# renegade-fi/mpc-jellyfish

Measured on AMD Instinct MI355X. Metric: msm_g1_scalar_pairs_per_s, higher is better.
Workload: dtype u32 (381-bit Fq as 14 x 29-bit limbs, Montgomery)

## Files before the change

mpc-jellyfish_amd/csrc/constants.cuh:

```cuda
#pragma once
#include <cstdint>

namespace mzk {

struct BlsFr {
    static constexpr int N = 8;
    static constexpr int BITS = 255;
    static constexpr uint32_t INV = 0xffffffffu;
    static constexpr uint32_t MOD[8] = {0x00000001u, 0xffffffffu, 0xfffe5bfeu, 0x53bda402u, 0x09a1d805u, 0x3339d808u, 0x299d7d48u, 0x73eda753u};
    static constexpr uint32_t R1[8] = {0xfffffffeu, 0x00000001u, 0x00034802u, 0x5884b7fau, 0xecbc4ff5u, 0x998c4fefu, 0xacc5056fu, 0x1824b159u};
    static constexpr uint32_t R2[8] = {0xf3f29c6du, 0xc999e990u, 0x87925c23u, 0x2b6cedcbu, 0x7254398fu, 0x05d31496u, 0x9f59ff11u, 0x0748d9d9u};
    static constexpr uint32_t ROOT[8] = {0x5f0e466au, 0xb9b58d8cu, 0x1819d7ecu, 0x5b1b4c80u, 0x52a31e64u, 0x0af53ae3u, 0x19e9b27bu, 0x5bf3addau};
    static constexpr uint32_t GENERATOR[8] = {0xfffffff1u, 0x0000000eu, 0x00189c0fu, 0x17e363d3u, 0x6f8457b0u, 0xff9c5787u, 0x8fc5a8c4u, 0x35133220u};
    static constexpr int TWO_ADICITY = 32;
};

struct BnFr {
    static constexpr int N = 8;
    static constexpr int BITS = 254;
    static constexpr uint32_t INV = 0xefffffffu;
    static constexpr uint32_t MOD[8] = {0xf0000001u, 0x43e1f593u, 0x79b97091u, 0x2833e848u, 0x8181585du, 0xb85045b6u, 0xe131a029u, 0x30644e72u};
    static constexpr uint32_t R1[8] = {0x4ffffffbu, 0xac96341cu, 0x9f60cd29u, 0x36fc7695u, 0x7879462eu, 0x666ea36fu, 0x9a07df2fu, 0x0e0a77c1u};
    static constexpr uint32_t R2[8] = {0xae216da7u, 0x1bb8e645u, 0xe35c59e3u, 0x53fe3ab1u, 0x53bb8085u, 0x8c49833du, 0x7f4e44a5u, 0x0216d0b1u};
    static constexpr uint32_t ROOT[8] = {0x80d13d9cu, 0x636e7355u, 0x2445ffd6u, 0xa22bf374u, 0x1eb203d8u, 0x56452ac0u, 0x2963f9e7u, 0x1860ef94u};
// ... 106 lines not shown
    static constexpr uint32_t XR2[9] = {0x059bac10u, 0x0d1503a3u, 0x018016b8u, 0x10ab0ca8u, 0x02632639u, 0x02c0169fu, 0x169bfd53u, 0x11869d4cu, 0x002a11a6u};
    static constexpr uint32_t XPINV[9] = {0x1b799c77u, 0x016fc3e8u, 0x0d654d9eu, 0x030535c2u, 0x0257f612u, 0x1a17f3e6u, 0x0e509d40u, 0x090dceeeu, 0x100a85ddu};
    static constexpr uint32_t XRM[8] = {0x0f6b5c04u, 0x751d5b0fu, 0xe6d91549u, 0x5edd77f4u, 0x422a9d60u, 0x1422c907u, 0xd2402342u, 0x1982b46du};
    static constexpr long long SRC = 346695ll;
    static constexpr int XPAD_MULT = 1;
    static constexpr uint32_t XSUB2[9] = {0x30f9fa8eu, 0x2208c16cu, 0x38e5469du, 0x25aa45a0u, 0x2b0bb2efu, 0x25b68180u, 0x214dc281u, 0x3cb84c67u, 0x0060c89bu};
    static constexpr uint32_t XSUB8[9] = {0x43e7ea38u, 0x482305b4u, 0x43951a76u, 0x56a91685u, 0x4c2ecbbeu, 0x56da0603u, 0x45370a06u, 0x52e1319eu, 0x01832271u};
    static constexpr uint32_t XSUB32[9] = {0x8f9fa8e0u, 0x808c16d4u, 0x8e5469ddu, 0x9aa45a18u, 0x90bb2efeu, 0x9b681811u, 0x94dc281eu, 0x8b84c67cu, 0x060c89cau};
    static constexpr uint32_t XSUB64[9] = {0x5f3f51c0u, 0x41182daeu, 0x5ca8d3c0u, 0x5548b436u, 0x41765e03u, 0x56d03029u, 0x49b85043u, 0x57098cffu, 0x0c19139au};
    static constexpr int XKXY = 8;
    static constexpr uint32_t XSUB_XY[9] = {0x43e7ea38u, 0x482305b4u, 0x43951a76u, 0x56a91685u, 0x4c2ecbbeu, 0x56da0603u, 0x45370a06u, 0x52e1319eu, 0x01832271u};
    static constexpr uint32_t XSUB_PQ[9] = {0x81f3f51cu, 0x841182d7u, 0x91ca8d38u, 0x8b548b3fu, 0x961765dcu, 0x8b6d02feu, 0x829b8500u, 0x997098ccu, 0x00c19135u};
    static constexpr uint32_t XSUB_2S[9] = {0x41f3f51cu, 0x441182d9u, 0x51ca8d3au, 0x4b548b41u, 0x561765deu, 0x4b6d0300u, 0x429b8502u, 0x597098ceu, 0x00c19137u};
};

}
```

mpc-jellyfish_amd/csrc/gen_constants.py:

```python
import os

FIELDS = {}

def limbs32(x, n):
    return [(x >> (32 * i)) & 0xFFFFFFFF for i in range(n)]

def carr(name, vals):
    return "    static constexpr uint32_t %s[%d] = {%s};" % (name, len(vals), ", ".join("0x%08xu" % v for v in vals))

def field_struct(name, p, n32, extra=(), tail=()):
    R = 1 << (32 * n32)
    out = ["struct %s {" % name,
           "    static constexpr int N = %d;            // 32-bit limbs" % n32,
           "    static constexpr int BITS = %d;" % p.bit_length(),
           "    static constexpr uint32_t INV = 0x%08xu;  // -p^-1 mod 2^32" % ((-pow(p, -1, 1 << 32)) % (1 << 32)),
           carr("MOD", limbs32(p, n32)),
           carr("R1", limbs32(R % p, n32)) + "   // Montgomery one",
           carr("R2", limbs32(R * R % p, n32)) + "   // R^2 mod p"]
    for k, v in extra:
        out.append(carr(k, limbs32(v * R % p, n32)))
    out.extend(tail)
    out.append("};")
    return "\n".join(out)

# ... 72 lines not shown
    out.append("    static constexpr int XKXY = %d;           // accumulator invariant: X, Y < XKXY * p" % kxy)
    out.append(arr("XSUB_XY", spread(kxy, p, n29, 1), "%dp: minus an accumulator coordinate (limbs < 2^30 - 1)" % kxy))
    out.append(arr("XSUB_PQ", spread(kpq, p, n29, 2), "%dp: minus PPP + 2Q (limbs < 2^31 - 3)" % kpq))
    out.append(arr("XSUB_2S", spread(k2s, p, n29, 1), "%dp: minus 2S (limbs < 2^30 - 1)" % k2s))
    out.append("};")
    return "\n".join(out)

out.append(fx_struct("BlsFrX", "BlsFr", bls_r, 8, 9))
out.append("")
out.append(fx_struct("BnFrX", "BnFr", bn_r, 8, 9))
out.append("")
out.append(fx_struct("BlsFqX", "BlsFq", bls_q, 12, 14, endo_beta=pow(2, (bls_q - 1) // 3, bls_q)))
out.append("")
out.append(fx_struct("BnFqX", "BnFq", bn_q, 8, 9, ec_pads=(8, 4, 4)))
out.append("")
out.append("}  // namespace mzk")
open(os.path.join(os.path.dirname(os.path.abspath(__file__)), "constants.cuh"), "w").write("\n".join(out) + "\n")
print("wrote constants.cuh")
```

mpc-jellyfish_amd/csrc/msm.cuh:

```cuda
#pragma once
#include <hip/hip_runtime.h>

#include "ec.cuh"
#include "ecx.cuh"

namespace mzk {

constexpr int MSM_THREADS = 256;
constexpr int MSM_ACC_THREADS = 128;
constexpr uint32_t MSM_HEAVY_PER_THREAD = 16;
constexpr uint32_t MSM_HEAVY_RUN = MSM_ACC_THREADS * MSM_HEAVY_PER_THREAD;
constexpr uint32_t MSM_HEAVY_FANIN = MSM_ACC_THREADS * 32;
constexpr int MSM_HEAVY_COUNTERS = 6;
__host__ __device__ inline bool msm_is_heavy(uint32_t count, uint32_t cap) { return count > cap + MSM_HEAVY_RUN; }

inline int msm_choose_window(unsigned long long n) {
    int lg = 0;
    while ((1ull << (lg + 1)) <= n) lg++;
    int c = lg - 2;
    if (c < 4) c = 4;
    if (c > 16) c = 16;
    return c;
}
inline int msm_num_windows(int scalar_bits, int c) { return (scalar_bits + 1 + c - 1) / c; }
// ... 240 lines not shown
};

template <class X>
__device__ __forceinline__ void load_words(uint32_t* dst, const uint32_t* __restrict__ src, int n_words) {
    for (int i = 0; i < n_words / 4; i++) {
        const uint4 v = reinterpret_cast<const uint4*>(src)[i];
        dst[4 * i] = v.x; dst[4 * i + 1] = v.y; dst[4 * i + 2] = v.z; dst[4 * i + 3] = v.w;
    }
}

template <class X>
struct EcFx {
    using Field = X;
    using Aff = AffineX<X>;
    using Pt = XYZZX<X>;
    static constexpr int AFF_WORDS = 2 * X::XN, PT_WORDS = 4 * X::XN;
    static_assert((4 * X::XN) % 4 == 0 && (2 * X::XN) % 2 == 0, "points are whole 16-byte / 8-byte words");
    static __device__ __forceinline__ Aff load_aff(const uint32_t* __restrict__ bases, unsigned long long idx) {
        uint32_t w[AFF_WORDS];
        if constexpr (AFF_WORDS % 4 == 0) {
            const uint4* src = reinterpret_cast<const uint4*>(bases + idx * AFF_WORDS);
#pragma unroll
            for (int i = 0; i < AFF_WORDS / 4; i++) {
                const uint4 v = src[i];
                w[4 * i] = v.x; w[4 * i + 1] = v.y; w[4 * i + 2] = v.z; w[4 * i + 3] = v.w;
            }
        } else {
            const uint2* src = reinterpret_cast<const uint2*>(bases + idx * AFF_WORDS);
#pragma unroll
            for (int i = 0; i < AFF_WORDS / 2; i++) {
// ... 23 lines not shown
    }
    static __device__ __forceinline__ void store_pt(uint32_t* __restrict__ buf, unsigned long long idx, const Pt& p) {
        uint32_t w[PT_WORDS];
#pragma unroll
        for (int i = 0; i < X::XN; i++) {
            w[i] = p.x.l[i]; w[X::XN + i] = p.y.l[i]; w[2 * X::XN + i] = p.zz.l[i]; w[3 * X::XN + i] = p.zzz.l[i];
        }
        uint4* dst = reinterpret_cast<uint4*>(buf + idx * PT_WORDS);
#pragma unroll
        for (int i = 0; i < PT_WORDS / 4; i++) dst[i] = make_uint4(w[4 * i], w[4 * i + 1], w[4 * i + 2], w[4 * i + 3]);
    }
    static __device__ __forceinline__ Pt inf() { return Pt::inf(); }
    static __device__ __forceinline__ Pt madd(const Pt& a, const Aff& q, bool negate) { return xyzzx_madd(a, q, negate); }
    static __device__ __forceinline__ Pt add(const Pt& a, const Pt& b) { return xyzzx_add(a, b); }
    static __device__ __forceinline__ XYZZ<Fp<X>> to_boundary(const Pt& p) { return xyzzx_to_boundary(p); }
};

template <class X>
__global__ __launch_bounds__(MSM_THREADS) void srs_to_internal_kernel(const uint32_t* __restrict__ xy, unsigned long long n, uint32_t* __restrict__ out) {
    const unsigned long long i = (unsigned long long)blockIdx.x * MSM_THREADS + threadIdx.x;
    if (i >= n) return;
    const Fp<X> x = load_fp<X>(xy + i * 2 * X::N), y = load_fp<X>(xy + i * 2 * X::N + X::N);
    const Fx<X> fx = fx_from_boundary<X>(x), fy = fx_from_boundary<X>(y);
    uint32_t* dst = out + i * 2 * X::XN;
#pragma unroll
    for (int k = 0; k < X::XN; k++) { dst[k] = fx.l[k]; dst[X::XN + k] = fy.l[k]; }
}

template <class EC>
__global__ __launch_bounds__(MSM_ACC_THREADS) void msm_accumulate_kernel(const uint32_t* __restrict__ bases, unsigned long long n,
                                                                          const uint32_t* __restrict__ offs, const uint32_t* __restrict__ hist,
// ... 44 lines not shown
    typename EC::Pt acc = EC::inf();
    for (uint32_t k = part; k < cnt; k += S) {
        const uint32_t e = list[k];
        acc = EC::madd(acc, EC::load_aff(bases, e & 0x7fffffffu), (e >> 31) != 0);
    }
    if (whole) {
        const bool empty = acc.is_inf();
        occ[t] = empty ? 0 : 1;
        if (!empty) EC::store_pt(buckets, t, acc);
    } else {
        EC::store_pt(sub, u, acc);
    }
}
template <class EC>
__device__ __forceinline__ void pt_lds_put(uint32_t* lds, int slot, const typename EC::Pt& p) {
    constexpr int N = EC::Field::XN;
#pragma unroll
    for (int i = 0; i < N; i++) {
        lds[i * MSM_ACC_THREADS + slot] = p.x.l[i];
        lds[(N + i) * MSM_ACC_THREADS + slot] = p.y.l[i];
        lds[(2 * N + i) * MSM_ACC_THREADS + slot] = p.zz.l[i];
        lds[(3 * N + i) * MSM_ACC_THREADS + slot] = p.zzz.l[i];
    }
}
template <class EC>
__device__ __forceinline__ typename EC::Pt pt_lds_get(const uint32_t* lds, int slot) {
    constexpr int N = EC::Field::XN;
    typename EC::Pt p;
#pragma unroll
    for (int i = 0; i < N; i++) {
        p.x.l[i] = lds[i * MSM_ACC_THREADS + slot];
        p.y.l[i] = lds[(N + i) * MSM_ACC_THREADS + slot];
        p.zz.l[i] = lds[(2 * N + i) * MSM_ACC_THREADS + slot];
        p.zzz.l[i] = lds[(3 * N + i) * MSM_ACC_THREADS + slot];
    }
    return p;
}
template <class EC, bool ONE_SET>
__global__ __launch_bounds__(MSM_ACC_THREADS) void msm_split_combine_kernel(const uint32_t* __restrict__ sub, unsigned long long n_buckets, int log_split,
                                                                             const uint32_t* __restrict__ order, unsigned long long rank0,
                                                                             uint32_t* __restrict__ buckets, uint8_t* __restrict__ occ) {
    __shared__ uint32_t lds[MSM_ACC_THREADS * EC::PT_WORDS];
// ... 317 lines not shown
        const uint32_t h = M >> lvl;
        const uint32_t items = (uint32_t)lvl * h;
        for (uint32_t r = threadIdx.x; r < items; r += 256) {
            const uint32_t seg = r / h, i = r % h;
            const unsigned long long base = w * M + (seg ? (M >> seg) : 0u);
            fold_one<EC>(buckets, occ, base + i, base + h + i);
        }
        __threadfence_block();
        __syncthreads();
    }
    if (collect && (int)threadIdx.x <= log_m) collect_set<EC>(buckets, occ, M, log_m, w, collect, (int)threadIdx.x);
}

template <class EC>
__device__ __forceinline__ void fold_one_quad(uint32_t* buckets, uint8_t* occ, unsigned long long ia, unsigned long long ib, int role) {
    using X = typename EC::Field;
    constexpr int XN = X::XN;
    if (!occ[ib]) return;
    uint32_t* pa = buckets + ia * EC::PT_WORDS + role * XN;
    const uint32_t* pb = buckets + ib * EC::PT_WORDS + role * XN;
    Fx<X> cb;
#pragma unroll
    for (int i = 0; i < XN; i++) cb.l[i] = pb[i];
    if (!occ[ia]) {
#pragma unroll
        for (int i = 0; i < XN; i++) pa[i] = cb.l[i];
        occ[ia] = 1;
        return;
    }
    Fx<X> ca;
#pragma unroll
    for (int i = 0; i < XN; i++) ca.l[i] = pa[i];
    const Fx<X> r = xyzzx_add_quad<X>(ca, cb, role);
#pragma unroll
    for (int i = 0; i < XN; i++) pa[i] = r.l[i];
}
template <class EC>
__global__ __launch_bounds__(MSM_ACC_THREADS) void msm_fold_quad_kernel(uint32_t* buckets, uint8_t* occ, uint32_t M, uint32_t h, int nseg, int n_win) {
    const unsigned long long t = ((unsigned long long)blockIdx.x * MSM_ACC_THREADS + threadIdx.x) >> 2;
    const int role = threadIdx.x & 3;
    const unsigned long long per_win = (unsigned long long)nseg * h;
    if (t >= per_win * n_win) return;
    const unsigned long long w = t / per_win, r = t % per_win;
    const uint32_t seg = (uint32_t)(r / h), i = (uint32_t)(r % h);
    const unsigned long long base = w * M + (seg ? (M >> seg) : 0u);
    fold_one_quad<EC>(buckets, occ, base + i, base + h + i, role);
}
constexpr int MSM_TAIL_QUAD_THREADS = 512;
// ... 287 lines not shown
```

mpc-jellyfish_amd/csrc/msm.hip:

```cpp
#include <algorithm>
#include <chrono>
#include <thread>
#include <vector>

#include <cmath>
#include <cstdlib>

#include "internal.hpp"
#include "hostfp.hpp"
#include "host_tail.hpp"
#include "msm.cuh"
#include "msm_pre.cuh"

namespace mzk {
std::atomic<bool> g_msm_precompute{true};
namespace {

struct MsmItem {
    const uint32_t* d_bases;
    const uint32_t* d_scalars;
    uint64_t n;
    uint32_t* out_xyz;
    uint64_t base_off;
};
// ... 491 lines not shown
        if (!p0)
            for (auto& it : run) it.d_bases = plain_table + it.base_off * aff_words;
        for (int attempt = 0;; attempt++) {
            const int32_t rc = msm_group_dev<FR, EC>(run.data(), j - i, c, is_mont, p0 ? pre : PreInfo{}, st);
            cur().last_attempts = (uint32_t)attempt + 1;
            if (rc == MSM_RETRY && attempt < 8) continue;
            if (rc == MSM_RETRY) { set_error("MSM heavy-bucket scratch: no fit after 8 attempts"); return MZK_ERR_UNSUPPORTED; }
            MZK_TRY(rc);
            break;
        }
        i = j;
    }
    return MZK_OK;
}

template <class X>
int32_t srs_build_pre_t(Srs& s, hipStream_t st) {
    using EC = EcFx<X>;
    int lg = 0;
    while ((2ull << lg) <= s.n) lg++;
    int c;
    if (s.curve == MZK_CURVE_BLS12_381) c = lg <= 17 ? 16 : 20;
    else c = lg <= 15 ? 15 : (lg <= 19 ? 17 : 20);
    if (const char* force = std::getenv("MZK_PRE_C")) {
        const int f = std::atoi(force);
        if (f >= 8 && f <= 22) c = f;
    }
    const int W = msm_num_windows(256, c);
    const size_t level = (size_t)s.n * EC::AFF_WORDS;
    size_t free_b = 0, total_b = 0;
    HIP_TRY(hipMemGetInfo(&free_b, &total_b));
    size_t budget = free_b / 2;
    if (const char* b = std::getenv("MZK_MSM_TABLE_BUDGET")) budget = std::min<size_t>(budget, (size_t)std::strtoull(b, nullptr, 10));
    if ((size_t)W * level * 4 > budget) { s.pre_c = -1; return MZK_OK; }
    HIP_TRY(hipMalloc((void**)&s.d_pre, (size_t)W * level * 4));
    HIP_TRY(hipStreamSynchronize(st));
    const auto t_build = std::chrono::steady_clock::now();
    HIP_TRY(hipMemcpyAsync(s.d_pre, s.d_int, level * 4, hipMemcpyDeviceToDevice, st));
    const unsigned long long threads = (s.n + 3) / 4;
    for (int w = 1; w < W; w++)
        hipLaunchKernelGGL((pre_next_level_kernel<X>), dim3((unsigned)((threads + 127) / 128)), dim3(128), 0, st,
                           s.d_pre + (size_t)(w - 1) * level, s.d_pre + (size_t)w * level, (unsigned long long)s.n, c);
    HIP_TRY(hipGetLastError());
    HIP_TRY(hipStreamSynchronize(st));
    s.pre_build_ms = std::chrono::duration<double, std::milli>(std::chrono::steady_clock::now() - t_build).count();
    s.pre_c = c;
    s.pre_levels = W;
    return MZK_OK;
}
}
int32_t srs_build_pre(Srs& s, hipStream_t st) {
    if (s.d_pre || s.pre_c < 0 || !s.d_int) return MZK_OK;
    return s.curve == MZK_CURVE_BLS12_381 ? srs_build_pre_t<BlsFqX>(s, st) : srs_build_pre_t<BnFqX>(s, st);
}

int32_t msm_dispatch(const Srs& s, uint64_t base_offset, const uint32_t* d_scalars, uint64_t n, int is_mont, uint32_t* out, hipStream_t st) {
    const uint32_t* sc[1] = {d_scalars};
    return msm_batch_dispatch(s, 1, sc, &n, &base_offset, is_mont, out, st);
}

int32_t msm_batch_dispatch(const Srs& s, uint32_t n_polys, const uint32_t* const* d_scalars, const uint64_t* lens, const uint64_t* base_offsets,
                           int is_mont, uint32_t* out_xyz, hipStream_t st) {
    const int fw = fq_words(s.curve);
    const bool bls = s.curve == MZK_CURVE_BLS12_381;
    const size_t aff_words = bls ? (size_t)EcFx<BlsFqX>::AFF_WORDS : (size_t)EcFx<BnFqX>::AFF_WORDS;
    const uint32_t* table = s.d_int;
    if (!table) { set_error("SRS has no internal table"); return MZK_ERR_BAD_HANDLE; }
    std::vector<MsmItem> items(n_polys);
    bool want_pre = false;
    for (uint32_t i = 0; i < n_polys; i++) {
        const uint64_t off = base_offsets ? base_offsets[i] : 0;
        if (off > s.n || lens[i] > s.n - off) {
            set_error("MSM longer than the registered SRS (poly degree larger than allowed)");
            return MZK_ERR_INVALID_ARG;
        }
        want_pre |= lens[i] >= PRE_MIN_N;
        items[i] = MsmItem{nullptr, d_scalars[i], lens[i], out_xyz + (size_t)i * 3 * fw, off};
    }
    PreInfo pre;
    if (want_pre && g_msm_precompute) {
        Srs& ms = const_cast<Srs&>(s);
        MZK_TRY(srs_build_pre(ms, st));
        if (ms.d_pre && ms.pre_c > 0) { pre.c = ms.pre_c; pre.tab_stride = ms.n; }
    }
    if (pre.c)
        for (auto& it : items) it.d_bases = s.d_pre;
    if (bls) return msm_batch_dev<BlsFr, EcFx<BlsFqX>>(items.data(), (int)n_polys, is_mont, pre, table, aff_words, st);
    return msm_batch_dev<BnFr, EcFx<BnFqX>>(items.data(), (int)n_polys, is_mont, pre, table, aff_words, st);
}

static_assert(srs_int_point_bytes(MZK_CURVE_BLS12_381) == EcFx<BlsFqX>::AFF_WORDS * 4 && srs_int_point_bytes(MZK_CURVE_BN254) == EcFx<BnFqX>::AFF_WORDS * 4,
              "srs_int_point_bytes (internal.hpp) is the size of an EcFx affine point");
template <class X>
static int32_t srs_build_internal_t(Srs& s, hipStream_t st) {
    using EC = EcFx<X>;
    HIP_TRY(hipMalloc((void**)&s.d_int, (size_t)(s.n ? s.n : 1) * EC::AFF_WORDS * 4));
    if (s.n) {
        hipLaunchKernelGGL((srs_to_internal_kernel<X>), dim3((unsigned)((s.n + MSM_THREADS - 1) / MSM_THREADS)), dim3(MSM_THREADS), 0, st,
                           s.d_xy, s.n, s.d_int);
        HIP_TRY(hipGetLastError());
        HIP_TRY(hipStreamSynchronize(st));
    }
    return MZK_OK;
}
int32_t srs_build_internal(Srs& s, hipStream_t st) {
    s.d_int = nullptr;
    s.d_pre = nullptr;
    s.pre_c = 0;
    return s.curve == MZK_CURVE_BLS12_381 ? srs_build_internal_t<BlsFqX>(s, st) : srs_build_internal_t<BnFqX>(s, st);
}

namespace {
template <class FR, class FQ>
int32_t srs_generate(const uint32_t* beta_canon, const uint32_t* g_xy_mont, uint64_t n, uint32_t* d_out) {
    hipStream_t st = nullptr;
    WsHold ws; MZK_TRY(ws.acquire(st));
    MZK_TRY(ws->scalars.reserve((n ? n : 1) * 32));
    MZK_TRY(ws->misc.reserve(32 + 256 * 4 * FQ::N * 4 + 256 * 2 * FQ::N * 4 + 2 * FQ::N * 4));
    uint32_t* d_beta = ws->misc.as<uint32_t>();
    uint32_t* d_tab_xyzz = d_beta + 8;
    uint32_t* d_tab = d_tab_xyzz + 256 * 4 * FQ::N;
    uint32_t* d_g = d_tab + 256 * 2 * FQ::N;
    HIP_TRY(hipMemcpyAsync(d_beta, beta_canon, 32, hipMemcpyHostToDevice, st));
    if (g_xy_mont) HIP_TRY(hipMemcpyAsync(d_g, g_xy_mont, 2 * FQ::N * 4, hipMemcpyHostToDevice, st));
// ... 153 lines not shown
```

mpc-jellyfish_amd/csrc/msm_pre.cuh:

```cuda
#pragma once
#include "msm.cuh"

namespace mzk {

constexpr int PRE_CHUNK = 4096;
inline uint32_t pre_chunk_of(unsigned long long n) {
    uint32_t chunk = PRE_CHUNK;
    while (chunk > 256 && n / chunk < 128) chunk >>= 1;
    return chunk;
}
constexpr int PRE_CTHREADS = 1024;
constexpr int PRE_FINE_LOG = 11;
constexpr uint32_t PRE_EMPTY = 0xFFFFFFFFu;

struct PreBins {
    uint32_t low, low_log, low_bins;
    uint32_t hi_log;
    __host__ __device__ uint32_t bin_of(uint32_t b) const { return b < low ? b >> low_log : low_bins + ((b - low) >> hi_log); }
    __host__ __device__ uint32_t first_bucket(uint32_t bin) const { return bin < low_bins ? bin << low_log : low + ((bin - low_bins) << hi_log); }
    __host__ __device__ uint32_t size_of(uint32_t bin, uint32_t M) const {
        const uint32_t full = bin < low_bins ? 1u << low_log : 1u << hi_log;
        const uint32_t left = M - first_bucket(bin);
        return full < left ? full : left;
    }
// ... 340 lines not shown
    for (int j = B - 1; j >= 0; j--) {
        if (start + j >= n) continue;
        uint32_t* dst = next + (start + j) * EC::AFF_WORDS;
        if (pt[j].is_inf()) {
            for (int k = 0; k < EC::AFF_WORDS; k++) dst[k] = 0;
            continue;
        }
        const Fx<X> zi = fx_mul(inv_run, pref[j]);
        inv_run = fx_mul(inv_run, pt[j].zzz);
        const Fx<X> zzi = fx_sqr(fx_mul(zi, pt[j].zz));
        const Fx<X> x = fx_canonical(fx_mul(pt[j].x, zzi)), y = fx_canonical(fx_mul(pt[j].y, zi));
#pragma unroll
        for (int k = 0; k < X::XN; k++) { dst[k] = x.l[k]; dst[X::XN + k] = y.l[k]; }
    }
}

}
```

Measured before the change: 335.0 million.

## Use signed 13x30-bit limb Montgomery arithmetic for BLS12-381 G1 MSM

Adds a new field representation for BLS12-381 Fq that uses 13 signed 30-bit limbs with lazy normalization, along with matching XYZZ point formulas, quad-lane add, SRS conversion and precompute kernels. The BLS MSM path now uses this representation in place of the 14x29-bit one. Fewer limbs cut the number of multiply-accumulates per Montgomery product and the register footprint. The cost is more sign-extension and rounding work, plus correctness risk from the signed bounds and a changed internal point size.

New measurement: 349.5 million, median of 6. +4.3%, better.

```diff
diff --git a/mpc-jellyfish_amd/csrc/constants.cuh b/mpc-jellyfish_amd/csrc/constants.cuh
--- a/mpc-jellyfish_amd/csrc/constants.cuh
+++ b/mpc-jellyfish_amd/csrc/constants.cuh
@@ -144,4 +144,17 @@
     static constexpr uint32_t XSUB_2S[9] = {0x41f3f51cu, 0x441182d9u, 0x51ca8d3au, 0x4b548b41u, 0x561765deu, 0x4b6d0300u, 0x429b8502u, 0x597098ceu, 0x00c19137u};
 };
 
+struct BlsFqZ : BlsFq {
+    static constexpr int ZN = 13;
+    static constexpr int ZL = 30;
+    static constexpr uint32_t ZINV = 0x3ffcfffdu;
+    static constexpr int ZHEADROOM_BITS = 9;
+    static constexpr int32_t ZP[13] = {-21845, -402915328, 356515836, -352321620, -252304353, 55215067, 288093811, 316751073, -321428361, 517541167, -375082566, -91332614, 1704210};
+    static constexpr int32_t ZPU[13] = {1073719979, 670826495, 356515835, 721420204, 821437470, 55215066, 288093811, 316751073, 752313463, 517541166, 698659258, 982409209, 1704209};
+    static constexpr int32_t ZONE[13] = {13762350, 433586176, -192935228, -301937177, 37952645, -425753694, -36732706, 162803105, -437337492, 366579475, 78814996, -442511456, 89578};
+    static constexpr int32_t ZR2[13] = {84936463, -82245875, 20063291, -375672600, -184045713, -75371400, -508475920, 172522421, -150322876, 98350284, 415856896, -132992156, 1010031};
+    static constexpr int32_t ZTO[13] = {-192885889, -32767999, -532500185, -13403472, -35343150, 503405810, 6050829, -194530918, -181768796, 433626394, -273043482, -129447912, 620336};
+    static constexpr int32_t ZFROM[13] = {196605, 405012480, 12582951, -50330895, 123255532, -496935601, -445360651, 370465813, -328370226, -362903204, 154517618, -251748295, 1439327};
+};
+
 }
diff --git a/mpc-jellyfish_amd/csrc/ecz.cuh b/mpc-jellyfish_amd/csrc/ecz.cuh
--- /dev/null
+++ b/mpc-jellyfish_amd/csrc/ecz.cuh
@@ -0,0 +1,190 @@
+#pragma once
+#include "ecx.cuh"
+#include "fz.cuh"
+
+namespace mzk {
+
+template <class Z>
+struct AffineZ {
+    Fz<Z> x, y;
+    MZK_HD bool is_inf() const {
+        int32_t a = 0;
+#pragma unroll
+        for (int i = 0; i < Z::ZN; i++) a |= x.l[i] | y.l[i];
+        return a == 0;
+    }
+};
+
+template <class Z>
+struct XYZZZ {
+    Fz<Z> x, y, zz, zzz;
+    MZK_HD bool is_inf() const { return fz_is_zero(zz); }
+    MZK_HD static XYZZZ inf() {
+        XYZZZ r;
+        r.x = Fz<Z>::one(); r.y = Fz<Z>::one(); r.zz = Fz<Z>::zero(); r.zzz = Fz<Z>::zero();
+        return r;
+    }
+    MZK_HD static XYZZZ from_affine(const AffineZ<Z>& p) {
+        if (p.is_inf()) return inf();
+        XYZZZ r;
+        r.x = p.x; r.y = p.y; r.zz = Fz<Z>::one(); r.zzz = Fz<Z>::one();
+        return r;
+    }
+};
+
+template <class Z>
+MZK_HD void ecz_xy3(Fz<Z>& x3, Fz<Z>& y3, const Fz<Z>& a, const Fz<Z>& b_plus_2c, const Fz<Z>& q, const Fz<Z>& r, const Fz<Z>& y, const Fz<Z>& ppp) {
+    x3 = fz_norm_wide(fz_sub(a, b_plus_2c));
+    const Fz<Z> d = fz_norm(fz_sub(q, x3));
+    y3 = fz_mul2(r, d, y, fz_neg(ppp));
+}
+
+template <class Z>
+MZK_HD XYZZZ<Z> xyzzz_dbl_affine(const AffineZ<Z>& p) {
+    XYZZZ<Z> r;
+    const Fz<Z> u = fz_norm(fz_add(p.y, p.y));
+    const Fz<Z> v = fz_sqr(u);
+    const Fz<Z> w = fz_mul(u, v);
+    const Fz<Z> s = fz_mul(p.x, v);
+    const Fz<Z> x2 = fz_sqr(p.x);
+    const Fz<Z> m = fz_norm_wide(fz_add(fz_add(x2, x2), x2));
+    const Fz<Z> mm = fz_sqr(m);
+    ecz_xy3<Z>(r.x, r.y, mm, fz_add(s, s), s, m, p.y, w);
+    r.zz = v;
+    r.zzz = w;
+    return r;
+}
+
+template <class Z>
+MZK_HD XYZZZ<Z> xyzzz_dbl(const XYZZZ<Z>& p) {
+    if (p.is_inf()) return p;
+    XYZZZ<Z> r;
+    const Fz<Z> u = fz_norm(fz_add(p.y, p.y));
+    const Fz<Z> v = fz_sqr(u);
+    const Fz<Z> w = fz_mul(u, v);
+    const Fz<Z> s = fz_mul(p.x, v);
+    const Fz<Z> x2 = fz_sqr(p.x);
+    const Fz<Z> m = fz_norm_wide(fz_add(fz_add(x2, x2), x2));
+    const Fz<Z> mm = fz_sqr(m);
+    ecz_xy3<Z>(r.x, r.y, mm, fz_add(s, s), s, m, p.y, w);
+    r.zz = fz_mul(v, p.zz);
+    r.zzz = fz_mul(w, p.zzz);
+    return r;
+}
+
+template <class Z>
+MZK_HD XYZZZ<Z> xyzzz_madd(const XYZZZ<Z>& p, const AffineZ<Z>& q, bool negate) {
+    if (q.is_inf()) return p;
+    const Fz<Z> qy = negate ? fz_neg(q.y) : q.y;
+    if (p.is_inf()) {
+        XYZZZ<Z> r;
+        r.x = q.x; r.y = qy; r.zz = Fz<Z>::one(); r.zzz = Fz<Z>::one();
+        return r;
+    }
+    const Fz<Z> u2 = fz_mul(q.x, p.zz);
+    const Fz<Z> s2 = fz_mul(qy, p.zzz);
+    const Fz<Z> pp_ = fz_norm(fz_sub(u2, p.x));
+    const Fz<Z> rr_ = fz_norm(fz_sub(s2, p.y));
+    const Fz<Z> pp = fz_sqr(pp_);
+    const Fz<Z> rr2 = fz_sqr(rr_);
+    if (fz_is_zero(pp)) {
+        if (fz_is_zero(rr2)) {
+            AffineZ<Z> qq;
+            qq.x = q.x;
+            qq.y = qy;
+            return xyzzz_dbl_affine(qq);
+        }
+        return XYZZZ<Z>::inf();
+    }
+    XYZZZ<Z> r;
+    const Fz<Z> ppp = fz_mul(pp_, pp);
+    const Fz<Z> qv = fz_mul(p.x, pp);
+    ecz_xy3<Z>(r.x, r.y, rr2, fz_add(ppp, fz_add(qv, qv)), qv, rr_, p.y, ppp);
+    r.zz = fz_mul(p.zz, pp);
+    r.zzz = fz_mul(p.zzz, ppp);
+    return r;
+}
+
+template <class Z>
+MZK_HD XYZZZ<Z> xyzzz_add(const XYZZZ<Z>& p, const XYZZZ<Z>& q) {
+    if (q.is_inf()) return p;
+    if (p.is_inf()) return q;
+    const Fz<Z> u1 = fz_mul(p.x, q.zz), u2 = fz_mul(q.x, p.zz);
+    const Fz<Z> s1 = fz_mul(p.y, q.zzz), s2 = fz_mul(q.y, p.zzz);
+    const Fz<Z> pp_ = fz_norm(fz_sub(u2, u1));
+    const Fz<Z> rr_ = fz_norm(fz_sub(s2, s1));
+    const Fz<Z> pp = fz_sqr(pp_);
+    const Fz<Z> rr2 = fz_sqr(rr_);
+    if (fz_is_zero(pp)) {
+        if (fz_is_zero(rr2)) return xyzzz_dbl(p);
+        return XYZZZ<Z>::inf();
+    }
+    XYZZZ<Z> r;
+    const Fz<Z> ppp = fz_mul(pp_, pp);
+    const Fz<Z> qv = fz_mul(u1, pp);
+    ecz_xy3<Z>(r.x, r.y, rr2, fz_add(ppp, fz_add(qv, qv)), qv, rr_, s1, ppp);
+    r.zz = fz_mul(fz_mul(p.zz, q.zz), pp);
+    r.zzz = fz_mul(fz_mul(p.zzz, q.zzz), ppp);
+    return r;
+}
+
+#if defined(__HIPCC__)
+template <int CTRL, class Z>
+__device__ __forceinline__ Fz<Z> fz_quad_perm(const Fz<Z>& a) {
+    Fz<Z> r;
+#pragma unroll
+    for (int i = 0; i < Z::ZN; i++) {
+        r.l[i] = __builtin_amdgcn_update_dpp(0, a.l[i], CTRL, 0xF, 0xF, true);
+        asm("" : "+v"(r.l[i]));
+    }
+    return r;
+}
+template <class Z>
+__device__ __forceinline__ Fz<Z> fz_sel(bool c, const Fz<Z>& a, const Fz<Z>& b) {
+    Fz<Z> r;
+#pragma unroll
+    for (int i = 0; i < Z::ZN; i++) r.l[i] = c ? a.l[i] : b.l[i];
+    return r;
+}
+
+template <class Z>
+__device__ __forceinline__ Fz<Z> xyzzz_add_quad(const Fz<Z>& ca, const Fz<Z>& cb, int role) {
+    const bool r0 = role == 0, r1 = role == 1, hi = role >= 2;
+    int special = (role == 2 && (fz_is_zero(ca) || fz_is_zero(cb))) ? 1 : 0;
+    const Fz<Z> p1 = fz_mul(ca, fz_quad_perm<QP_SWAP2>(cb));
+    const Fz<Z> d = fz_norm(fz_sub(fz_quad_perm<QP_SWAP2>(p1), p1));
+    const Fz<Z> p2 = fz_mul(fz_sel(hi, ca, d), fz_sel(hi, cb, d));
+    if (r0 && fz_is_zero(p2)) special = 1;
+    special |= __builtin_amdgcn_update_dpp(0, special, QP_SWAP1, 0xF, 0xF, true);
+    special |= __builtin_amdgcn_update_dpp(0, special, QP_SWAP2, 0xF, 0xF, true);
+    if (special) {
+        XYZZZ<Z> a, b;
+        a.x = fz_quad_perm<QP_L0>(ca); a.y = fz_quad_perm<QP_L1>(ca); a.zz = fz_quad_perm<QP_L2>(ca); a.zzz = fz_quad_perm<QP_L3>(ca);
+        b.x = fz_quad_perm<QP_L0>(cb); b.y = fz_quad_perm<QP_L1>(cb); b.zz = fz_quad_perm<QP_L2>(cb); b.zzz = fz_quad_perm<QP_L3>(cb);
+        const XYZZZ<Z> r = xyzzz_add(a, b);
+        return fz_sel(hi, fz_sel(role == 2, r.zz, r.zzz), fz_sel(r0, r.x, r.y));
+    }
+    const Fz<Z> pp = fz_quad_perm<QP_L0>(p2);
+    const Fz<Z> u1 = fz_quad_perm<QP_L0>(p1);
+    const Fz<Z> p3 = fz_mul(fz_sel(r0, d, fz_sel(r1, u1, p2)), pp);
+    const Fz<Z> ppp = fz_quad_perm<QP_L0>(p3);
+    const Fz<Z> x3 = fz_norm_wide(fz_sub(p2, fz_add(ppp, fz_add(p3, p3))));
+    const Fz<Z> qx = fz_norm(fz_sub(p3, x3));
+    const Fz<Z> s1 = fz_quad_perm<QP_L1>(p1);
+    const Fz<Z> p4 = fz_mul(fz_sel(r0, s1, fz_sel(r1, d, p2)), fz_sel(r1, qx, ppp));
+    const Fz<Z> y3 = fz_norm(fz_sub(p4, fz_quad_perm<QP_L0>(p4)));
+    const Fz<Z> x3_0 = fz_quad_perm<QP_L1>(x3);
+    return fz_sel(hi, fz_sel(role == 2, p3, p4), fz_sel(r0, x3_0, y3));
+}
+#endif
+
+template <class Z>
+MZK_HD XYZZ<Fp<Z>> xyzzz_to_boundary(const XYZZZ<Z>& p) {
+    XYZZ<Fp<Z>> r;
+    if (p.is_inf()) return XYZZ<Fp<Z>>::inf();
+    r.x = fz_to_boundary<Z>(p.x); r.y = fz_to_boundary<Z>(p.y);
+    r.zz = fz_to_boundary<Z>(p.zz); r.zzz = fz_to_boundary<Z>(p.zzz);
+    return r;
+}
+
+}
diff --git a/mpc-jellyfish_amd/csrc/fz.cuh b/mpc-jellyfish_amd/csrc/fz.cuh
--- /dev/null
+++ b/mpc-jellyfish_amd/csrc/fz.cuh
@@ -0,0 +1,287 @@
+#pragma once
+#include "fp.cuh"
+
+namespace mzk {
+
+template <class Z>
+struct Fz {
+    static constexpr int N = Z::ZN;
+    int32_t l[N];
+    MZK_HD static Fz zero() {
+        Fz r;
+#pragma unroll
+        for (int i = 0; i < N; i++) r.l[i] = 0;
+        return r;
+    }
+    MZK_HD static Fz from_const(const int32_t (&c)[Z::ZN]) {
+        Fz r;
+#pragma unroll
+        for (int i = 0; i < N; i++) r.l[i] = c[i];
+        return r;
+    }
+    MZK_HD static Fz one() { return from_const(Z::ZONE); }
+};
+
+MZK_HD int32_t fz_sext(uint32_t v) { return (int32_t)(v << 2) >> 2; }
+template <class Z>
+MZK_HD int32_t fz_p_limb(int i) {
+    int32_t v = Z::ZP[i];
+#if defined(__HIP_DEVICE_COMPILE__)
+    asm("" : "+s"(v));
+#endif
+    return v;
+}
+
+template <class Z>
+MZK_HD Fz<Z> fz_mul(const Fz<Z>& x, const Fz<Z>& y) {
+    constexpr int N = Z::ZN;
+    int32_t m[N], pl[N];
+#pragma unroll
+    for (int i = 0; i < N; i++) pl[i] = fz_p_limb<Z>(i);
+    Fz<Z> t;
+    int64_t acc = 0;
+#pragma unroll
+    for (int k = 0; k < N; k++) {
+#pragma unroll
+        for (int i = 0; i <= k; i++) acc += (int64_t)x.l[i] * y.l[k - i];
+#pragma unroll
+        for (int i = 0; i < k; i++) acc += (int64_t)m[i] * pl[k - i];
+        m[k] = fz_sext((uint32_t)acc * Z::ZINV);
+        acc += (int64_t)m[k] * pl[0];
+        acc >>= Z::ZL;
+    }
+#pragma unroll
+    for (int k = N; k < 2 * N - 1; k++) {
+#pragma unroll
+        for (int i = k - N + 1; i < N; i++) {
+            acc += (int64_t)x.l[i] * y.l[k - i];
+            acc += (int64_t)m[i] * pl[k - i];
+        }
+        t.l[k - N] = fz_sext((uint32_t)acc);
+        acc = (acc + (1 << (Z::ZL - 1))) >> Z::ZL;
+    }
+    t.l[N - 1] = (int32_t)acc;
+    return t;
+}
+template <class Z>
+MZK_HD Fz<Z> fz_mul2(const Fz<Z>& x, const Fz<Z>& y, const Fz<Z>& u, const Fz<Z>& v) {
+    constexpr int N = Z::ZN;
+    int32_t m[N], pl[N];
+#pragma unroll
+    for (int i = 0; i < N; i++) pl[i] = fz_p_limb<Z>(i);
+    Fz<Z> t;
+    int64_t acc = 0;
+#pragma unroll
+    for (int k = 0; k < N; k++) {
+#pragma unroll
+        for (int i = 0; i <= k; i++) {
+            acc += (int64_t)x.l[i] * y.l[k - i];
+            acc += (int64_t)u.l[i] * v.l[k - i];
+        }
+#pragma unroll
+        for (int i = 0; i < k; i++) acc += (int64_t)m[i] * pl[k - i];
+        m[k] = fz_sext((uint32_t)acc * Z::ZINV);
+        acc += (int64_t)m[k] * pl[0];
+        acc >>= Z::ZL;
+    }
+#pragma unroll
+    for (int k = N; k < 2 * N - 1; k++) {
+#pragma unroll
+        for (int i = k - N + 1; i < N; i++) {
+            acc += (int64_t)x.l[i] * y.l[k - i];
+            acc += (int64_t)u.l[i] * v.l[k - i];
+            acc += (int64_t)m[i] * pl[k - i];
+        }
+        t.l[k - N] = fz_sext((uint32_t)acc);
+        acc = (acc + (1 << (Z::ZL - 1))) >> Z::ZL;
+    }
+    t.l[N - 1] = (int32_t)acc;
+    return t;
+}
+template <class Z>
+MZK_HD Fz<Z> fz_sqr(const Fz<Z>& x) {
+    constexpr int N = Z::ZN;
+    int32_t m[N], pl[N], x2[N];
+#pragma unroll
+    for (int i = 0; i < N; i++) { pl[i] = fz_p_limb<Z>(i); x2[i] = x.l[i] * 2; }
+    Fz<Z> t;
+    int64_t acc = 0;
+#pragma unroll
+    for (int k = 0; k < N; k++) {
+#pragma unroll
+        for (int i = 0; 2 * i < k; i++) acc += (int64_t)x.l[i] * x2[k - i];
+        if (k % 2 == 0) acc += (int64_t)x.l[k / 2] * x.l[k / 2];
+#pragma unroll
+        for (int i = 0; i < k; i++) acc += (int64_t)m[i] * pl[k - i];
+        m[k] = fz_sext((uint32_t)acc * Z::ZINV);
+        acc += (int64_t)m[k] * pl[0];
+        acc >>= Z::ZL;
+    }
+#pragma unroll
+    for (int k = N; k < 2 * N - 1; k++) {
+#pragma unroll
+        for (int i = k - N + 1; 2 * i < k; i++) acc += (int64_t)x.l[i] * x2[k - i];
+        if (k % 2 == 0) acc += (int64_t)x.l[k / 2] * x.l[k / 2];
+#pragma unroll
+        for (int i = k - N + 1; i < N; i++) acc += (int64_t)m[i] * pl[k - i];
+        t.l[k - N] = fz_sext((uint32_t)acc);
+        acc = (acc + (1 << (Z::ZL - 1))) >> Z::ZL;
+    }
+    t.l[N - 1] = (int32_t)acc;
+    return t;
+}
+
+template <class Z>
+MZK_HD Fz<Z> fz_add(const Fz<Z>& a, const Fz<Z>& b) {
+    Fz<Z> r;
+#pragma unroll
+    for (int i = 0; i < Z::ZN; i++) r.l[i] = a.l[i] + b.l[i];
+    return r;
+}
+template <class Z>
+MZK_HD Fz<Z> fz_sub(const Fz<Z>& a, const Fz<Z>& b) {
+    Fz<Z> r;
+#pragma unroll
+    for (int i = 0; i < Z::ZN; i++) r.l[i] = a.l[i] - b.l[i];
+    return r;
+}
+template <class Z>
+MZK_HD Fz<Z> fz_neg(const Fz<Z>& a) {
+    Fz<Z> r;
+#pragma unroll
+    for (int i = 0; i < Z::ZN; i++) r.l[i] = -a.l[i];
+    return r;
+}
+
+template <class Z>
+MZK_HD Fz<Z> fz_norm(const Fz<Z>& a) {
+    constexpr int N = Z::ZN, L = Z::ZL;
+    Fz<Z> r;
+    r.l[0] = fz_sext((uint32_t)a.l[0]);
+#pragma unroll
+    for (int i = 1; i < N - 1; i++) r.l[i] = fz_sext((uint32_t)a.l[i]) + ((a.l[i - 1] + (1 << (L - 1))) >> L);
+    r.l[N - 1] = a.l[N - 1] + ((a.l[N - 2] + (1 << (L - 1))) >> L);
+    return r;
+}
+template <class Z>
+MZK_HD Fz<Z> fz_norm_wide(const Fz<Z>& a) {
+    constexpr int N = Z::ZN, L = Z::ZL;
+    Fz<Z> r;
+    r.l[0] = fz_sext((uint32_t)a.l[0]);
+#pragma unroll
+    for (int i = 1; i < N - 1; i++) r.l[i] = fz_sext((uint32_t)a.l[i]) + (((a.l[i - 1] >> (L - 1)) + 1) >> 1);
+    r.l[N - 1] = a.l[N - 1] + (((a.l[N - 2] >> (L - 1)) + 1) >> 1);
+    return r;
+}
+template <class Z>
+MZK_HD Fz<Z> fz_carry(const Fz<Z>& a) {
+    constexpr int N = Z::ZN, L = Z::ZL;
+    Fz<Z> r;
+    int32_t c = 0;
+#pragma unroll
+    for (int i = 0; i < N - 1; i++) {
+        const int32_t t = a.l[i] + c;
+        r.l[i] = fz_sext((uint32_t)t);
+        c = ((t >> (L - 1)) + 1) >> 1;
+    }
+    r.l[N - 1] = a.l[N - 1] + c;
+    return r;
+}
+template <class Z>
+MZK_HD bool fz_is_zero(const Fz<Z>& a) {
+    int32_t z = 0;
+#pragma unroll
+    for (int i = 0; i < Z::ZN; i++) z |= a.l[i];
+    return z == 0;
+}
+template <class Z>
+MZK_HD Fz<Z> fz_canonical(const Fz<Z>& a) {
+    constexpr int N = Z::ZN, L = Z::ZL;
+    constexpr int32_t MASK = (1 << L) - 1;
+    Fz<Z> r;
+    int32_t c = 0;
+#pragma unroll
+    for (int i = 0; i < N - 1; i++) {
+        const int32_t t = a.l[i] + c;
+        r.l[i] = t & MASK;
+        c = t >> L;
+    }
+    r.l[N - 1] = a.l[N - 1] + c;
+    const bool negative = r.l[N - 1] < 0;
+    Fz<Z> s;
+    c = 0;
+#pragma unroll
+    for (int i = 0; i < N - 1; i++) {
+        const int32_t t = r.l[i] + Z::ZPU[i] + c;
+        s.l[i] = t & MASK;
+        c = t >> L;
+    }
+    s.l[N - 1] = r.l[N - 1] + Z::ZPU[N - 1] + c;
+#pragma unroll
+    for (int i = 0; i < N; i++) r.l[i] = negative ? s.l[i] : r.l[i];
+    return r;
+}
+
+template <class Z>
+MZK_HD Fz<Z> fz_unpack(const uint32_t* w) {
+    constexpr int N = Z::ZN, W = Z::N, L = Z::ZL;
+    Fz<Z> r;
+#pragma unroll
+    for (int i = 0; i < N; i++) {
+        const int bit = L * i, wi = bit >> 5, s = bit & 31;
+        uint32_t v = wi < W ? (w[wi] >> s) : 0u;
+        if (s > 32 - L && wi + 1 < W) v |= w[wi + 1] << (32 - s);
+        r.l[i] = (int32_t)(v & ((1u << L) - 1));
+    }
+    return fz_carry(r);
+}
+template <class Z>
+MZK_HD void fz_pack(uint32_t* w, const Fz<Z>& a) {
+    constexpr int N = Z::ZN, W = Z::N, L = Z::ZL;
+#pragma unroll
+    for (int j = 0; j < W; j++) {
+        const int bit = 32 * j, i0 = bit / L, o = bit - L * i0;
+        uint32_t v = i0 < N ? (uint32_t)a.l[i0] >> o : 0u;
+        if (i0 + 1 < N) v |= (uint32_t)a.l[i0 + 1] << (L - o);
+        if (2 * L - o < 32 && i0 + 2 < N) v |= (uint32_t)a.l[i0 + 2] << (2 * L - o);
+        w[j] = v;
+    }
+}
+
+template <class Z>
+MZK_HD Fz<Z> fz_from_boundary(const Fp<Z>& a) {
+    return fz_mul(fz_unpack<Z>(a.l), Fz<Z>::from_const(Z::ZTO));
+}
+template <class Z>
+MZK_HD Fp<Z> fz_to_boundary(const Fz<Z>& a) {
+    Fp<Z> r;
+    fz_pack<Z>(r.l, fz_canonical(fz_mul(a, Fz<Z>::from_const(Z::ZFROM))));
+    return r;
+}
+
+template <class Z>
+MZK_HD Fz<Z> fz_inv(const Fz<Z>& a) {
+    Fz<Z> tab[16];
+    tab[0] = Fz<Z>::one();
+    tab[1] = fz_mul(a, tab[0]);
+#pragma unroll 1
+    for (int i = 2; i < 16; i++) tab[i] = fz_mul(tab[i - 1], tab[1]);
+    uint32_t e[Z::N];
+#pragma unroll
+    for (int i = 0; i < Z::N; i++) e[i] = Z::MOD[i];
+    uint32_t borrow = e[0] < 2 ? 1u : 0u;
+    e[0] -= 2;
+#pragma unroll
+    for (int i = 1; i < Z::N; i++) { const uint32_t t = e[i]; e[i] = t - borrow; borrow = (borrow && t == 0) ? 1u : 0u; }
+    Fz<Z> acc = tab[0];
+#pragma unroll 1
+    for (int d = 8 * Z::N - 1; d >= 0; d--) {
+#pragma unroll 1
+        for (int k = 0; k < 4; k++) acc = fz_sqr(acc);
+        const uint32_t nib = (e[d >> 3] >> ((d & 7) * 4)) & 15u;
+        if (nib) acc = fz_mul(acc, tab[nib]);
+    }
+    return acc;
+}
+
+}
diff --git a/mpc-jellyfish_amd/csrc/gen_constants.py b/mpc-jellyfish_amd/csrc/gen_constants.py
--- a/mpc-jellyfish_amd/csrc/gen_constants.py
+++ b/mpc-jellyfish_amd/csrc/gen_constants.py
@@ -110,6 +110,42 @@
 out.append("")
 out.append(fx_struct("BnFqX", "BnFq", bn_q, 8, 9, ec_pads=(8, 4, 4)))
 out.append("")
+
+L30 = 30
+def balanced30(x, n):
+    d = []
+    for _ in range(n - 1):
+        v = x & ((1 << L30) - 1)
+        if v >= 1 << (L30 - 1):
+            v -= 1 << L30
+        d.append(v)
+        x = (x - v) >> L30
+    d.append(x)
+    assert -(1 << 29) <= x < (1 << 29)
+    return d
+
+def fz_struct(name, base, p, n32, n30):
+    R = 1 << (32 * n32)
+    Rp = 1 << (L30 * n30)
+    out = ["struct %s : %s {" % (name, base),
+           "    static constexpr int ZN = %d;             // signed 30-bit limbs, R' = 2^(30*ZN)" % n30,
+           "    static constexpr int ZL = %d;" % L30,
+           "    static constexpr uint32_t ZINV = 0x%08xu;   // -p^-1 mod 2^30" % ((-pow(p, -1, 1 << L30)) % (1 << L30)),
+           "    static constexpr int ZHEADROOM_BITS = %d;  // 30*ZN - bits(p)" % (L30 * n30 - p.bit_length())]
+    def arr(nm, vals, cmt=""):
+        return "    static constexpr int32_t %s[%d] = {%s};%s" % (nm, len(vals), ", ".join("%d" % v for v in vals), ("   // " + cmt) if cmt else "")
+    bal = balanced30(p, n30)
+    out.append(arr("ZP", bal, "p, balanced limbs (sum of |limb| = %.2f * 2^29)" % (sum(abs(v) for v in bal) / 2.0 ** 29)))
+    out.append(arr("ZPU", [(p >> (L30 * i)) & ((1 << L30) - 1) for i in range(n30)], "p, limbs in [0, 2^30) (fz_canonical)"))
+    out.append(arr("ZONE", balanced30(Rp % p, n30), "R' mod p: the internal one"))
+    out.append(arr("ZR2", balanced30(Rp * Rp % p, n30), "R'^2: fz_mul(x, ZR2) = x*R' for an integer x"))
+    out.append(arr("ZTO", balanced30(Rp * Rp * pow(R, -1, p) % p, n30), "R'^2/R: fz_mul(x*R, ZTO) = x*R'"))
+    out.append(arr("ZFROM", balanced30(R % p, n30), "R: fz_mul(x*R', ZFROM) = x*R"))
+    out.append("};")
+    return "\n".join(out)
+
+out.append(fz_struct("BlsFqZ", "BlsFq", bls_q, 12, 13))
+out.append("")
 out.append("}  // namespace mzk")
 open(os.path.join(os.path.dirname(os.path.abspath(__file__)), "constants.cuh"), "w").write("\n".join(out) + "\n")
 print("wrote constants.cuh")
diff --git a/mpc-jellyfish_amd/csrc/msm.cuh b/mpc-jellyfish_amd/csrc/msm.cuh
--- a/mpc-jellyfish_amd/csrc/msm.cuh
+++ b/mpc-jellyfish_amd/csrc/msm.cuh
@@ -3,6 +3,7 @@
 
 #include "ec.cuh"
 #include "ecx.cuh"
+#include "ecz.cuh"
 
 namespace mzk {
 
@@ -278,6 +279,8 @@
     using Field = X;
     using Aff = AffineX<X>;
     using Pt = XYZZX<X>;
+    using Fe = Fx<X>;
+    static constexpr int LIMBS = X::XN, SLOT_WORDS = X::XN;
     static constexpr int AFF_WORDS = 2 * X::XN, PT_WORDS = 4 * X::XN;
     static_assert((4 * X::XN) % 4 == 0 && (2 * X::XN) % 2 == 0, "points are whole 16-byte / 8-byte words");
     static __device__ __forceinline__ Aff load_aff(const uint32_t* __restrict__ bases, unsigned long long idx) {
@@ -331,7 +334,86 @@
     static __device__ __forceinline__ Pt madd(const Pt& a, const Aff& q, bool negate) { return xyzzx_madd(a, q, negate); }
     static __device__ __forceinline__ Pt add(const Pt& a, const Pt& b) { return xyzzx_add(a, b); }
     static __device__ __forceinline__ XYZZ<Fp<X>> to_boundary(const Pt& p) { return xyzzx_to_boundary(p); }
+    static __device__ __forceinline__ Fe add_quad(const Fe& ca, const Fe& cb, int role) { return xyzzx_add_quad<X>(ca, cb, role); }
 };
+
+template <class Z>
+struct EcFz {
+    using Field = Z;
+    using Aff = AffineZ<Z>;
+    using Pt = XYZZZ<Z>;
+    using Fe = Fz<Z>;
+    static constexpr int LIMBS = Z::ZN, SLOT_WORDS = Z::ZN + 1;
+    static constexpr int AFF_WORDS = 2 * SLOT_WORDS, PT_WORDS = 4 * SLOT_WORDS;
+    static_assert(AFF_WORDS % 4 == 0, "points are whole 16-byte words");
+    static __device__ __forceinline__ Aff load_aff(const uint32_t* __restrict__ bases, unsigned long long idx) {
+        uint32_t w[AFF_WORDS];
+        const uint4* src = reinterpret_cast<const uint4*>(bases + idx * AFF_WORDS);
+#pragma unroll
+        for (int i = 0; i < AFF_WORDS / 4; i++) {
+            const uint4 v = src[i];
+            w[4 * i] = v.x; w[4 * i + 1] = v.y; w[4 * i + 2] = v.z; w[4 * i + 3] = v.w;
+        }
+        Aff p;
+#pragma unroll
+        for (int i = 0; i < LIMBS; i++) { p.x.l[i] = (int32_t)w[i]; p.y.l[i] = (int32_t)w[SLOT_WORDS + i]; }
+        return p;
+    }
+    static __device__ __forceinline__ void store_aff(uint32_t* __restrict__ bases, unsigned long long idx, const Aff& p) {
+        uint32_t w[AFF_WORDS];
+#pragma unroll
+        for (int i = 0; i < LIMBS; i++) { w[i] = (uint32_t)p.x.l[i]; w[SLOT_WORDS + i] = (uint32_t)p.y.l[i]; }
+        w[LIMBS] = 0; w[SLOT_WORDS + LIMBS] = 0;
+        uint4* dst = reinterpret_cast<uint4*>(bases + idx * AFF_WORDS);
+#pragma unroll
+        for (int i = 0; i < AFF_WORDS / 4; i++) dst[i] = make_uint4(w[4 * i], w[4 * i + 1], w[4 * i + 2], w[4 * i + 3]);
+    }
+    static __device__ __forceinline__ Pt load_pt(const uint32_t* __restrict__ buf, unsigned long long idx) {
+        uint32_t w[PT_WORDS];
+        const uint4* src = reinterpret_cast<const uint4*>(buf + idx * PT_WORDS);
+#pragma unroll
+        for (int i = 0; i < PT_WORDS / 4; i++) {
+            const uint4 v = src[i];
+            w[4 * i] = v.x; w[4 * i + 1] = v.y; w[4 * i + 2] = v.z; w[4 * i + 3] = v.w;
+        }
+        Pt p;
+#pragma unroll
+        for (int i = 0; i < LIMBS; i++) {
+            p.x.l[i] = (int32_t)w[i]; p.y.l[i] = (int32_t)w[SLOT_WORDS + i];
+            p.zz.l[i] = (int32_t)w[2 * SLOT_WORDS + i]; p.zzz.l[i] = (int32_t)w[3 * SLOT_WORDS + i];
+        }
+        return p;
+    }
+    static __device__ __forceinline__ void store_pt(uint32_t* __restrict__ buf, unsigned long long idx, const Pt& p) {
+        uint32_t w[PT_WORDS];
+#pragma unroll
+        for (int i = 0; i < LIMBS; i++) {
+            w[i] = (uint32_t)p.x.l[i]; w[SLOT_WORDS + i] = (uint32_t)p.y.l[i];
+            w[2 * SLOT_WORDS + i] = (uint32_t)p.zz.l[i]; w[3 * SLOT_WORDS + i] = (uint32_t)p.zzz.l[i];
+        }
+#pragma unroll
+        for (int k = 0; k < 4; k++) w[k * SLOT_WORDS + LIMBS] = 0;
+        uint4* dst = reinterpret_cast<uint4*>(buf + idx * PT_WORDS);
+#pragma unroll
+        for (int i = 0; i < PT_WORDS / 4; i++) dst[i] = make_uint4(w[4 * i], w[4 * i + 1], w[4 * i + 2], w[4 * i + 3]);
+    }
+    static __device__ __forceinline__ Pt inf() { return Pt::inf(); }
+    static __device__ __forceinline__ Pt madd(const Pt& a, const Aff& q, bool negate) { return xyzzz_madd(a, q, negate); }
+    static __device__ __forceinline__ Pt add(const Pt& a, const Pt& b) { return xyzzz_add(a, b); }
+    static __device__ __forceinline__ XYZZ<Fp<Z>> to_boundary(const Pt& p) { return xyzzz_to_boundary(p); }
+    static __device__ __forceinline__ Fe add_quad(const Fe& ca, const Fe& cb, int role) { return xyzzz_add_quad<Z>(ca, cb, role); }
+};
+
+template <class Z>
+__global__ __launch_bounds__(MSM_THREADS) void srs_to_internal_z_kernel(const uint32_t* __restrict__ xy, unsigned long long n, uint32_t* __restrict__ out) {
+    const unsigned long long i = (unsigned long long)blockIdx.x * MSM_THREADS + threadIdx.x;
+    if (i >= n) return;
+    const Fp<Z> x = load_fp<Z>(xy + i * 2 * Z::N), y = load_fp<Z>(xy + i * 2 * Z::N + Z::N);
+    AffineZ<Z> p;
+    p.x = fz_from_boundary<Z>(x);
+    p.y = fz_from_boundary<Z>(y);
+    EcFz<Z>::store_aff(out, i, p);
+}
 
 template <class X>
 __global__ __launch_bounds__(MSM_THREADS) void srs_to_internal_kernel(const uint32_t* __restrict__ xy, unsigned long long n, uint32_t* __restrict__ out) {
@@ -406,7 +488,7 @@
 }
 template <class EC>
 __device__ __forceinline__ void pt_lds_put(uint32_t* lds, int slot, const typename EC::Pt& p) {
-    constexpr int N = EC::Field::XN;
+    constexpr int N = EC::LIMBS;
 #pragma unroll
     for (int i = 0; i < N; i++) {
         lds[i * MSM_ACC_THREADS + slot] = p.x.l[i];
@@ -417,7 +499,7 @@
 }
 template <class EC>
 __device__ __forceinline__ typename EC::Pt pt_lds_get(const uint32_t* lds, int slot) {
-    constexpr int N = EC::Field::XN;
+    constexpr int N = EC::LIMBS;
     typename EC::Pt p;
 #pragma unroll
     for (int i = 0; i < N; i++) {
@@ -765,12 +847,12 @@
 
 template <class EC>
 __device__ __forceinline__ void fold_one_quad(uint32_t* buckets, uint8_t* occ, unsigned long long ia, unsigned long long ib, int role) {
-    using X = typename EC::Field;
-    constexpr int XN = X::XN;
+    using Fe = typename EC::Fe;
+    constexpr int XN = EC::LIMBS, SLOT = EC::SLOT_WORDS;
     if (!occ[ib]) return;
-    uint32_t* pa = buckets + ia * EC::PT_WORDS + role * XN;
-    const uint32_t* pb = buckets + ib * EC::PT_WORDS + role * XN;
-    Fx<X> cb;
+    uint32_t* pa = buckets + ia * EC::PT_WORDS + role * SLOT;
+    const uint32_t* pb = buckets + ib * EC::PT_WORDS + role * SLOT;
+    Fe cb;
 #pragma unroll
     for (int i = 0; i < XN; i++) cb.l[i] = pb[i];
     if (!occ[ia]) {
@@ -779,10 +861,10 @@
         occ[ia] = 1;
         return;
     }
-    Fx<X> ca;
+    Fe ca;
 #pragma unroll
     for (int i = 0; i < XN; i++) ca.l[i] = pa[i];
-    const Fx<X> r = xyzzx_add_quad<X>(ca, cb, role);
+    const Fe r = EC::add_quad(ca, cb, role);
 #pragma unroll
     for (int i = 0; i < XN; i++) pa[i] = r.l[i];
 }
diff --git a/mpc-jellyfish_amd/csrc/msm.hip b/mpc-jellyfish_amd/csrc/msm.hip
--- a/mpc-jellyfish_amd/csrc/msm.hip
+++ b/mpc-jellyfish_amd/csrc/msm.hip
@@ -529,9 +529,8 @@
     return MZK_OK;
 }
 
-template <class X>
-int32_t srs_build_pre_t(Srs& s, hipStream_t st) {
-    using EC = EcFx<X>;
+template <class EC>
+int32_t srs_build_pre_t(Srs& s, hipStream_t st, void (*next_level)(const uint32_t*, uint32_t*, unsigned long long, int)) {
     int lg = 0;
     while ((2ull << lg) <= s.n) lg++;
     int c;
@@ -554,7 +553,7 @@
     HIP_TRY(hipMemcpyAsync(s.d_pre, s.d_int, level * 4, hipMemcpyDeviceToDevice, st));
     const unsigned long long threads = (s.n + 3) / 4;
     for (int w = 1; w < W; w++)
-        hipLaunchKernelGGL((pre_next_level_kernel<X>), dim3((unsigned)((threads + 127) / 128)), dim3(128), 0, st,
+        hipLaunchKernelGGL(next_level, dim3((unsigned)((threads + 127) / 128)), dim3(128), 0, st,
                            s.d_pre + (size_t)(w - 1) * level, s.d_pre + (size_t)w * level, (unsigned long long)s.n, c);
     HIP_TRY(hipGetLastError());
     HIP_TRY(hipStreamSynchronize(st));
@@ -566,7 +565,8 @@
 }
 int32_t srs_build_pre(Srs& s, hipStream_t st) {
     if (s.d_pre || s.pre_c < 0 || !s.d_int) return MZK_OK;
-    return s.curve == MZK_CURVE_BLS12_381 ? srs_build_pre_t<BlsFqX>(s, st) : srs_build_pre_t<BnFqX>(s, st);
+    return s.curve == MZK_CURVE_BLS12_381 ? srs_build_pre_t<EcFz<BlsFqZ>>(s, st, pre_next_level_z_kernel<BlsFqZ>)
+                                          : srs_build_pre_t<EcFx<BnFqX>>(s, st, pre_next_level_kernel<BnFqX>);
 }
 
 int32_t msm_dispatch(const Srs& s, uint64_t base_offset, const uint32_t* d_scalars, uint64_t n, int is_mont, uint32_t* out, hipStream_t st) {
@@ -578,7 +578,7 @@
                            int is_mont, uint32_t* out_xyz, hipStream_t st) {
     const int fw = fq_words(s.curve);
     const bool bls = s.curve == MZK_CURVE_BLS12_381;
-    const size_t aff_words = bls ? (size_t)EcFx<BlsFqX>::AFF_WORDS : (size_t)EcFx<BnFqX>::AFF_WORDS;
+    const size_t aff_words = bls ? (size_t)EcFz<BlsFqZ>::AFF_WORDS : (size_t)EcFx<BnFqX>::AFF_WORDS;
     const uint32_t* table = s.d_int;
     if (!table) { set_error("SRS has no internal table"); return MZK_ERR_BAD_HANDLE; }
     std::vector<MsmItem> items(n_polys);
@@ -600,19 +600,18 @@
     }
     if (pre.c)
         for (auto& it : items) it.d_bases = s.d_pre;
-    if (bls) return msm_batch_dev<BlsFr, EcFx<BlsFqX>>(items.data(), (int)n_polys, is_mont, pre, table, aff_words, st);
+    if (bls) return msm_batch_dev<BlsFr, EcFz<BlsFqZ>>(items.data(), (int)n_polys, is_mont, pre, table, aff_words, st);
     return msm_batch_dev<BnFr, EcFx<BnFqX>>(items.data(), (int)n_polys, is_mont, pre, table, aff_words, st);
 }
 
-static_assert(srs_int_point_bytes(MZK_CURVE_BLS12_381) == EcFx<BlsFqX>::AFF_WORDS * 4 && srs_int_point_bytes(MZK_CURVE_BN254) == EcFx<BnFqX>::AFF_WORDS * 4,
-              "srs_int_point_bytes (internal.hpp) is the size of an EcFx affine point");
-template <class X>
-static int32_t srs_build_internal_t(Srs& s, hipStream_t st) {
-    using EC = EcFx<X>;
+static_assert(srs_int_point_bytes(MZK_CURVE_BLS12_381) == EcFz<BlsFqZ>::AFF_WORDS * 4 && srs_int_point_bytes(MZK_CURVE_BN254) == EcFx<BnFqX>::AFF_WORDS * 4,
+              "srs_int_point_bytes (internal.hpp) is the size of an internal affine point");
+template <class EC>
+static int32_t srs_build_internal_t(Srs& s, hipStream_t st, void (*to_internal)(const uint32_t*, unsigned long long, uint32_t*)) {
     HIP_TRY(hipMalloc((void**)&s.d_int, (size_t)(s.n ? s.n : 1) * EC::AFF_WORDS * 4));
     if (s.n) {
-        hipLaunchKernelGGL((srs_to_internal_kernel<X>), dim3((unsigned)((s.n + MSM_THREADS - 1) / MSM_THREADS)), dim3(MSM_THREADS), 0, st,
-                           s.d_xy, s.n, s.d_int);
+        hipLaunchKernelGGL(to_internal, dim3((unsigned)((s.n + MSM_THREADS - 1) / MSM_THREADS)), dim3(MSM_THREADS), 0, st,
+                           (const uint32_t*)s.d_xy, (unsigned long long)s.n, s.d_int);
         HIP_TRY(hipGetLastError());
         HIP_TRY(hipStreamSynchronize(st));
     }
@@ -622,7 +621,8 @@
     s.d_int = nullptr;
     s.d_pre = nullptr;
     s.pre_c = 0;
-    return s.curve == MZK_CURVE_BLS12_381 ? srs_build_internal_t<BlsFqX>(s, st) : srs_build_internal_t<BnFqX>(s, st);
+    return s.curve == MZK_CURVE_BLS12_381 ? srs_build_internal_t<EcFz<BlsFqZ>>(s, st, srs_to_internal_z_kernel<BlsFqZ>)
+                                          : srs_build_internal_t<EcFx<BnFqX>>(s, st, srs_to_internal_kernel<BnFqX>);
 }
 
 namespace {
diff --git a/mpc-jellyfish_amd/csrc/msm_pre.cuh b/mpc-jellyfish_amd/csrc/msm_pre.cuh
--- a/mpc-jellyfish_amd/csrc/msm_pre.cuh
+++ b/mpc-jellyfish_amd/csrc/msm_pre.cuh
@@ -378,5 +378,42 @@
         for (int k = 0; k < X::XN; k++) { dst[k] = x.l[k]; dst[X::XN + k] = y.l[k]; }
     }
 }
-
-}
+template <class Z>
+__global__ __launch_bounds__(128) void pre_next_level_z_kernel(const uint32_t* __restrict__ cur, uint32_t* __restrict__ next, unsigned long long n, int c) {
+    constexpr int B = 4;
+    using EC = EcFz<Z>;
+    const unsigned long long t = (unsigned long long)blockIdx.x * 128 + threadIdx.x;
+    const unsigned long long start = t * B;
+    if (start >= n) return;
+    XYZZZ<Z> pt[B];
+    Fz<Z> pref[B];
+    Fz<Z> run = Fz<Z>::one();
+#pragma unroll
+    for (int j = 0; j < B; j++) {
+        XYZZZ<Z> p = XYZZZ<Z>::inf();
+        if (start + j < n) {
+            p = XYZZZ<Z>::from_affine(EC::load_aff(cur, start + j));
+            for (int k = 0; k < c; k++) p = xyzzz_dbl(p);
+        }
+        pt[j] = p;
+        pref[j] = run;
+        if (!p.is_inf()) run = fz_mul(run, p.zzz);
+    }
+    Fz<Z> inv_run = fz_inv(run);
+#pragma unroll
+    for (int j = B - 1; j >= 0; j--) {
+        if (start + j >= n) continue;
+        AffineZ<Z> a;
+        a.x = Fz<Z>::zero(); a.y = Fz<Z>::zero();
+        if (!pt[j].is_inf()) {
+            const Fz<Z> zi = fz_mul(inv_run, pref[j]);
+            inv_run = fz_mul(inv_run, pt[j].zzz);
+            const Fz<Z> zzi = fz_sqr(fz_mul(zi, pt[j].zz));
+            a.x = fz_mul(pt[j].x, zzi);
+            a.y = fz_mul(pt[j].y, zi);
+        }
+        EC::store_aff(next, start + j, a);
+    }
+}
+
+}
```
